# flashlight/text

Hardware: AMD Instinct MI355X
Metric: decoded frames/sec (whole node), T=1000 N=29 beam=50; hyp bit-exact vs CPU (higher is better)
Workload: dtype f64; 1 GPU; C2: LexiconFreeDecoder + ZeroLM CTC, batch=256 utterances/GPU, T=1000, N=29, beam=50, beamToken=29, beamThreshold=25, logAdd=false, `ctc` emissions; parallelism=utterance-sharded x1, no collective, threads_per_utterance=512, lds_bytes_per_workgroup=16656, engine=4, redone=0, unread_redone=0, lane_groups=1, fallback_reasons=0

## Files before the change

### text_amd/csrc/fltx_api.cpp

```cpp
#include <algorithm>
#include <cmath>
#include <cstdarg>
#include <cstdio>
#include <cstdlib>
#include <cstring>
#include <thread>
#include <limits>
#include <map>
#include <memory>
#include <mutex>
#include <string>
#include <atomic>
#include <unordered_map>
#include <unordered_set>
#include <vector>

#include "fltx.h"
#include "fltx_kernel_entry.h"
#include "fltx_engines.h"
#include "fltx_s2s.h"
#include "fltx_s2s_lex.h"
#include "fltx_ctc_rows.h"
#include "fltx_ctc_rows_lex.h"
#include "fltx_ctc_rows_stream.h"
// ... 690 lines not shown
  DBuf scored;
  HBuf hlmQCount, hlmQ, hlmBeamN, hlmBeam, hlmStage;
  DBuf hlmTabD;
  int hlmQCap = 0;
  bool hlmAnnounce = false;
  int64_t hlmAsked = 0, hlmDistinct = 0;
  bool keepScored = false;
  int64_t idCap = 0;
  DBuf tokens, words, prof, histS, bestLen, bestScores, bestTok, bestWrd;
  HBuf hTokens, hWords, hScores;
  HBuf hTok8, hWordsC, hPackMeta;
  TrBufs tr;
  HBuf hSync;
  HBuf hStat;
  DBuf dTok8, dWordsC, dPackMeta;
  std::vector<int64_t> packOff;
  bool compactFetched = false, scoresFetched = false;
  DBuf uttMap;
  int nLaunch = 0;
  std::vector<int32_t> hLen, hNHyp;
  bool hostFetched = false;
  int keepScores = 0, userKeepScores = 0;
  int profile = 0, profWave = 0;
  std::vector<int32_t> hN, hFrame, hStatus;
  bool resultsSynced = false;
  bool backtraced = false;
  int64_t statFrames = 0, statBytes = 0, statDecodeBytes = 0, statEpilogueBytes = 0, statLmBytes = 0;
  bool statsDone = false;
#ifndef FLTX_EMU
  hipEvent_t ev[3] = {nullptr, nullptr, nullptr};
  hipStream_t copyStream = nullptr;
  hipEvent_t evSlotFree[2] = {nullptr, nullptr};
  bool slotUsed[2] = {false, false};
#endif
  bool timed = false;
  struct {
    fltx_s2s_options opt{};
    int eos = 0, maxOut = 0, t = 0, cap = 0, mSel = 0, eosExtra = 0;
    bool begun = false;
    int32_t ctx0[kS2sCtx] = {0};
    DBuf beam, beamN, hist, rowsInt, done, finalStep, recTok, recAm, recN, cKey;
    DBuf scores, valid;
    DBuf recLm, lmScores;
    int lmWidth = 0, lmFinish = 0;
    DBuf rowNode, lmRowOf;
    double wordScore = 0.0;
    bool isLmToken = false;
    int maxLabels = 0, slots = 1, mSize = 0, sSize = 0, sMax = 0, maxStates = 0;
    int64_t nodes = 0, edges = 0, labels = 0, trieBytes = 0;
    DBuf trieMax, kidOff, kidTok, kidNode, labOff, lab;
    DBuf cScore, cMk, cGrp, cList, cNext, mTab, sKey, sVal, sCount, status, merges;
    int crMaxT = 0;
    int64_t crFrames = 0;
    DBuf crMeta, crEmis;
    std::vector<int64_t> crMetaHost;
    const float* crEmisDev = nullptr;
    DBuf crOutBeam;
    bool crStream = false;
    int crCap = 0, crRing = 0, crBestLb = -1;
    std::vector<int32_t> crBestLen;
    std::vector<double> crBestScores;
    DBuf crCnt, crSHist;
    DBuf crIds, crMarks;
    std::vector<int32_t> crBuf;
    bool plOn = false, plFresh = false, plSkipped = false;
    int plRowCap = 0, plMetaPar = 0, plPrevPar = 0, plCollects = 0;
    DBuf plRowOf, plFree, plMeta, plPrev, plCnt, plRank;
// ... 971 lines not shown
  d->blank = blank;
  d->unk = unk;
  d->isLmToken = isLmToken ? 1 : 0;
  if (transitions && nTrans > 0) {
    d->nTrans = nTrans;
    d->transMax = 0.0;
    for (int i = 0; i < nTrans; ++i) {
      d->transMax = std::max(d->transMax, (double)transitions[i]);
    }
    if (d->transitions.ensure(sizeof(float) * (size_t)nTrans, ctx->stream, false) ||
        devCopyH2D(d->transitions.p, transitions, sizeof(float) * (size_t)nTrans, ctx->stream) ||
        devSync(ctx->stream)) {
      delete d;
      return fail(FLTX_ERR_HIP, "transitions upload failed");
    }
  }
  *out = d;
  return FLTX_OK;
}

int fltx_decoder_destroy(fltx_decoder* d) {
  DeviceScope devScope(d ? d->ctx : nullptr);
  if (devScope.failed) {
    return fail(FLTX_ERR_HIP, "hipSetDevice failed");
  }
  if (d) {
    devSync(d->ctx->stream);
#ifndef FLTX_EMU
    for (int i = 0; i < 3; ++i) {
      if (d->ev[i]) {
        (void)hipEventDestroy(d->ev[i]);
      }
    }
    if (d->copyStream) {
      (void)hipStreamSynchronize(d->copyStream);
      (void)hipEventDestroy(d->evSlotFree[0]);
      (void)hipEventDestroy(d->evSlotFree[1]);
      (void)hipStreamDestroy(d->copyStream);
    }
#endif
  }
  delete d;
  return FLTX_OK;
}

static int settlePendingLook(fltx_decoder* d);
static int trTimedSlot(const char* key) {
  static const char* const kKeys[4] = {"transcript_count_ns", "transcript_scan_ns", "transcript_write_ns", "pack_ns"};
  for (int i = 0; i < 4; ++i) {
    if (!strcmp(key, kKeys[i])) {
      return i;
    }
  }
  return -1;
}
static int btProfileGet(fltx_decoder* d, const char* what, int64_t* value) {
  if (!d->btProfile || !d->btProf.p || !d->backtraced) {
    return fail(FLTX_ERR_STATE, "no back-trace profile: fltx_decoder_set(dec, \"bt_profile\", 1) before the batch");
  }
  DeviceScope devScope(d->ctx);
  std::vector<unsigned long long> h((size_t)kBtProfMarks * d->B);
  if (devCopyD2H(h.data(), d->btProf.p, 8 * h.size(), d->ctx->stream)) {
    return fail(FLTX_ERR_HIP, "profile copy failed");
  }
  int64_t sum[8] = {0, 0, 0, 0, 0, 0, 0, 0};
  for (int b = 0; b < d->B; ++b) {
    const unsigned long long* m = h.data() + (size_t)b * kBtProfMarks;
    if (!m[1]) {
      continue;
    }
    sum[0] += (int64_t)(m[1] - m[0]);
    unsigned long long prev = m[1];
    for (int c = 0; c < (int)m[6]; ++c) {
      sum[1] += (int64_t)(m[8 + 2 * c] - prev);
      sum[2] += (int64_t)(m[9 + 2 * c] - m[8 + 2 * c]);
      prev = m[9 + 2 * c];
    }
    sum[1] += (int64_t)(m[2] - prev);
    sum[3] += (int64_t)(m[3] - m[2]);
    if (m[5]) {
      sum[4] += (int64_t)(m[4] - m[3]);
      sum[5] += (int64_t)(m[5] - m[4]);
    }
    sum[6] += (int64_t)((m[5] ? m[5] : m[3]) - m[0]);
    sum[7] += 1;
  }
  static const char* const kNames[8] = {"copy0", "walk", "wait", "store", "fetch0", "score", "total", "utts"};
  for (int i = 0; i < 8; ++i) {
    if (!strcmp(what, kNames[i])) {
      *value = sum[i];
      return FLTX_OK;
    }
  }
  return fail(FLTX_ERR_INVALID, "fltx_decoder_get: unknown key bt_prof_%s", what);
}

int fltx_decoder_get(fltx_decoder* d, const char* key, int64_t* value) {
  if (!d || !key || !value) {
    return fail(FLTX_ERR_INVALID, "fltx_decoder_get: null argument");
  }
  if (!strcmp(key, "engine")) {
    *value = d->engineFirst;
  } else if (!strcmp(key, "xlane")) {
    *value = d->xlaneFirst;
  } else if (!strcmp(key, "ylane")) {
    *value = d->ylaneFirst;
  } else if (!strcmp(key, "yshare")) {
    *value = (d->ylane || d->xlane) ? d->yshare : 0;
  } else if (!strcmp(key, "redone")) {
    if (d->offlinePending) {
      DeviceScope devScope(d->ctx);
      int rc = settlePendingLook(d);
      if (rc) {
        return rc;
      }
    }
    *value = d->lastRedo;
  } else if (!strcmp(key, "sstream")) {
    *value = d->sstream;
  } else if (!strcmp(key, "tstream")) {
    *value = d->tstream;
// ... 1333 lines not shown
int settleStream(fltx_decoder* d);
}
static int offlineAttempts(fltx_decoder* d, const float* emissions, int32_t onDevice, int firstAttempt);
namespace {

int syncResults(fltx_decoder* d) {
  if (!d->settling && (d->chunkPending || d->pendingPrune >= 0)) {
    int rc = settleStream(d);
    if (rc) {
      return rc;
    }
  }
  if (d->offlinePending) {
    d->offlinePending = false;
    d->upSlot = d->offUpSlot;
    int rc = offlineAttempts(d, d->offEmis, 1, 1);
    if (rc) {
      return rc;
    }
  }
  if (d->resultsSynced) {
    return FLTX_OK;
  }
  Stream st = d->ctx->stream;
  const int B = d->B;
  d->hN.resize(B);
  d->hFrame.resize(B);
  d->hStatus.resize(B);
  const size_t row = d->uttRow;
  if (d->hSync.ensure(4 * (2 * row + (size_t)B))) {
    return fail(FLTX_ERR_OOM, "pinned staging allocation failed");
  }
  const int32_t* h = (const int32_t*)d->hSync.p;
  if (devCopyD2H(d->hSync.p, d->uttRes.p, 4 * (2 * row + (size_t)B), st)) {
    return fail(FLTX_ERR_HIP, "result copy failed: %s", devErr());
  }
  memcpy(d->hN.data(), h, 4 * (size_t)B);
  memcpy(d->hFrame.data(), h + row, 4 * (size_t)B);
  memcpy(d->hStatus.data(), h + 2 * row, 4 * (size_t)B);
  d->resultsSynced = true;
  return FLTX_OK;
}

int launchBacktrace(fltx_decoder* d) {
  Stream st = d->ctx->stream;
  if (d->tokens.ensure(4 * (size_t)std::max<int64_t>(d->histRecords, 1), st, false)) {
    return fail(FLTX_ERR_OOM, "token buffer allocation failed");
  }
  if (d->kind == FLTX_DECODER_LEXICON &&
      d->words.ensure(4 * (size_t)std::max<int64_t>(d->histRecords, 1), st, false)) {
    return fail(FLTX_ERR_OOM, "word buffer allocation failed");
  }
  BacktraceParams Q;
  memset(&Q, 0, sizeof(Q));
  Q.K = d->opt.beam_size;
  Q.kind = d->kind;
  Q.histPT = d->histPT.as<int2>();
  Q.histW = d->histW.as<int32_t>();
  Q.histOff = d->histOffD.as<int64_t>();
  Q.uttFrame = d->uttFrame.as<int32_t>();
  Q.uttNBeam = d->uttNBeam.as<int32_t>();
  Q.tokOff = d->histOffD.as<int64_t>();
  Q.tokens = d->tokens.as<int32_t>();
  Q.words = d->kind == FLTX_DECODER_LEXICON ? d->words.as<int32_t>() : nullptr;
  Q.nbest = 0;
#ifdef FLTX_EMU
  const int btAsked = d->btThreads ? d->btThreads : 64;
// ... 27 lines not shown
  Q.F = F;
  size_t btLds = F > 0 ? (size_t)F * perFrame + 16 : 16;
  if (d->batchPacked && F > 0) {
    Q.packed = d->packedBits;
    Q.packedTokMask = d->batchWlane ? 0x7FFFFFFF : 0xFF;
    Q.amGather = d->batchWlane ? 1 : 0;
    Q.uttStatus = d->uttStatus.as<int32_t>();
    Q.amOut = d->outScores.as<double>();
    Q.emissions = d->lastEmis;
    Q.emOff = d->emOff[d->upSlot].as<int64_t>();
    Q.N = d->N;
    Q.transitions = (d->opt.criterion == FLTX_CRITERION_ASG && d->nTrans) ? d->transitions.as<float>() : nullptr;
    Q.tokLm = d->batchTlane ? d->tokLm : nullptr;
    Q.tokLmStride = d->N + 1;
    Q.blank = d->opt.criterion == FLTX_CRITERION_CTC ? d->blank : -1;
    const size_t amLds = Q.amGather ? 4 * (size_t)Q.K * F + 16
                                    : 4 * ((size_t)F * d->N + (Q.transitions ? (size_t)d->N * d->N : 0) + (size_t)Q.K * F) + 16;
    btLds = std::max(btLds, amLds);
  }
  int narrow = 0;
  int walkWaves = 1;
  if (d->batchPacked && F > 0 && Q.K <= btThreads) {
    const bool byteRec = d->packedBits <= 8 && Q.packedTokMask == 0xFF && d->N <= 255;
    const bool wordRec = d->packedBits <= 16 && d->N <= 65535;
    const size_t rec = byteRec ? 2 : 4, tokB = rec / 2;
    size_t row = 0;
    for (int b = 0; b < d->B; ++b) {
      row = std::max<size_t>(row, (size_t)((d->histOff[b + 1] - d->histOff[b]) / Q.K));
    }
    const bool lexRec = d->kind == FLTX_DECODER_LEXICON;
    const size_t tile = ((size_t)Q.K * row * tokB + 15) & ~(size_t)15;
    const size_t room = btBudget > tile + 16 ? btBudget - tile - 16 : 0;
    const size_t perWalk = (size_t)Q.K * (2 * rec + (lexRec ? 2 * 4 + 4 : 0));
    const size_t trBytes = (Q.transitions && !Q.amGather) ? 4 * (size_t)d->N * d->N : 0;
    const size_t perEm = 2 * 4 * (size_t)d->N;
    const size_t npF = std::min<size_t>(room / perWalk, std::max<size_t>(row, 8));
    const size_t npFe = Q.amGather ? (size_t)1 << 20 : (room > trBytes ? std::min<size_t>((room - trBytes) / perEm, std::max<size_t>(row, 8)) : 0);
    const size_t nW = (size_t)btThreads / 64;
    if ((byteRec || wordRec) && Q.K <= 64 && nW >= 2 && d->btWalkAsked != 1 && row > 0 && row < (1u << 24) && npF >= 8) {
      const size_t pwChunk = (((size_t)Q.K * npF * rec + 15) & ~(size_t)15) + (lexRec ? (size_t)Q.K * npF * (4 + 4) : 0);
      const size_t exitB = (nW * Q.K + 15) & ~(size_t)15;
      const size_t ent = ((size_t)Q.K * nW * ((row + npF - 1) / npF) + 15) & ~(size_t)15;
      const size_t roomE = room > ent ? room - ent : 0;
      const size_t perEmPw = (Q.amGather ? 0 : perEm) + 2 * (size_t)Q.K * tokB;
      const size_t pwFe = roomE > trBytes ? std::min<size_t>((roomE - trBytes) / perEmPw, std::max<size_t>(row, 8)) : 0;
      if (ent + exitB + pwChunk <= room && pwFe >= 8) {
        narrow = (int)rec;
        walkWaves = (int)nW;
        Q.npRow = (int32_t)row;
        Q.npF = (int32_t)npF;
        Q.npFe = (int32_t)pwFe;
        Q.npWaves = (int32_t)nW;
        Q.npEntry = (int32_t)tile;
        Q.npScratch = (int32_t)(tile + ent);
        btLds = std::max(btLds, tile + ent + std::max(exitB + pwChunk, trBytes + pwFe * perEmPw) + 16);
      }
    }
    if (!narrow && (byteRec || wordRec) && row > 0 && row < (1u << 24) && npF >= 8 && npFe >= 8) {
      narrow = (int)rec;
      Q.npRow = (int32_t)row;
      Q.npF = (int32_t)npF;
      Q.npFe = (int32_t)npFe;
      Q.npScratch = (int32_t)tile;
      btLds = std::max(btLds, tile + std::max(npF * perWalk, Q.amGather ? (size_t)0 : trBytes + npFe * perEm) + 16);
    }
  }
  if (narrow && d->btProfile) {
    if (d->btProf.ensure(8 * (size_t)kBtProfMarks * d->B, st, true)) {
      return fail(FLTX_ERR_OOM, "back-trace profile allocation failed");
    }
    devMemset(d->btProf.p, 0, 8 * (size_t)kBtProfMarks * d->B, st);
    Q.btProf = d->btProf.as<unsigned long long>();
  }
  d->btWalkWaves = walkWaves;
  d->btNarrow = narrow;
  d->btChunk = narrow ? Q.npF : F;
  d->btStretch = narrow ? (Q.amGather ? 0 : Q.npFe) : (d->batchPacked && !Q.amGather ? F : 0);
#ifdef FLTX_EMU
  const BacktraceParams* qq = &Q;
  if (narrow == 2 && walkWaves > 1) {
    emuLaunch(d->B, btThreads, btLds, [qq](char* smem) { backtraceNarrow<uint16_t, true>(*qq, smem); });
  } else if (narrow == 4 && walkWaves > 1) {
    emuLaunch(d->B, btThreads, btLds, [qq](char* smem) { backtraceNarrow<uint32_t, true>(*qq, smem); });
  } else if (narrow == 2) {
    emuLaunch(d->B, btThreads, btLds, [qq](char* smem) { backtraceNarrow<uint16_t, false>(*qq, smem); });
  } else if (narrow == 4) {
    emuLaunch(d->B, btThreads, btLds, [qq](char* smem) { backtraceNarrow<uint32_t, false>(*qq, smem); });
  } else {
    emuLaunch(d->B, btThreads, btLds, [qq](char* smem) { backtraceUtterance(*qq, smem); });
  }
#else
  const void* btFn = narrow == 2   ? (walkWaves > 1 ? (const void*)fltx_backtrace_narrow_kernel<uint16_t, true>
                                                   : (const void*)fltx_backtrace_narrow_kernel<uint16_t, false>)
                     : narrow == 4 ? (walkWaves > 1 ? (const void*)fltx_backtrace_narrow_kernel<uint32_t, true>
                                                   : (const void*)fltx_backtrace_narrow_kernel<uint32_t, false>)
                                   : (const void*)fltx_backtrace_kernel;
  int rcLds = raiseMaxLdsOnce(d, 1, btFn, btLds);
  if (rcLds) {
    return rcLds;
  }
  void* btArgs[] = {(void*)&Q};
  HIPCHK(hipLaunchKernel(btFn, dim3(d->B), dim3(btThreads), btArgs, btLds, st));
  HIPCHK(hipGetLastError());
  if (d->ev[2]) {
    HIPCHK(hipEventRecord(d->ev[2], st));
    d->timed = true;
  }
#endif
  d->backtraced = true;
  return FLTX_OK;
// ... 445 lines not shown
    return rc;
  }
  d->lastRedo = 0;
  d->resultsSynced = false;
  if ((rc = launchBacktrace(d))) {
    return rc;
  }
  d->T.assign(T, T + B);
  d->statsDone = false;
  d->haveResults = true;
  d->ended = true;
  return FLTX_OK;
}

}

extern "C" {

int fltx_decode_batch(fltx_decoder* d, const float* emissions, int32_t onDevice, const int64_t* offsets,
                      const int32_t* T, int32_t B, int32_t N) {
  DeviceScope devScope(d ? d->ctx : nullptr);
  if (devScope.failed) {
    return fail(FLTX_ERR_HIP, "hipSetDevice failed");
  }
  if (d && stepKindCalls(d->kind)) {
    return fail(FLTX_ERR_STATE, "fltx_decode_batch: %s", stepKindCalls(d->kind));
  }
  if (!d || !T || B <= 0 || N <= 0) {
    return fail(FLTX_ERR_INVALID, "fltx_decode_batch: bad argument");
  }
  if (d->offlinePending) {
    if (d->deferCheck == 2) {
      d->offlinePending = false;
      ++d->looksDropped;
    } else {
      int rc = syncResults(d);
      if (rc) {
        return rc;
      }
      d->unreadRedone += d->lastRedo;
    }
  }
  d->streaming = false;
  d->chunkPending = false;
  d->pendingPrune = -1;
  d->haveResults = false;
  d->resultsSynced = false;
  d->backtraced = false;
  d->hostFetched = false;
  d->compactFetched = false;
  d->scoresFetched = false;
  if (d->lm->kind == 2) {
    return hostLmDecodeBatch(d, emissions, onDevice, offsets, T, B, N);
  }
  d->offT.assign(T, T + B);
  d->offOffsets.clear();
  if (offsets) {
    d->offOffsets.assign(offsets, offsets + B);
  }
  d->offN = N;
  d->offlinePending = false;
  return offlineAttempts(d, emissions, onDevice, 0);
}

}
static int settlePendingLook(fltx_decoder* d) { return syncResults(d); }
static int offlineAttempts(fltx_decoder* d, const float* emissions, int32_t onDevice, int firstAttempt) {
  const int32_t* T = d->offT.data();
  const int64_t* offsets = d->offOffsets.empty() ? nullptr : d->offOffsets.data();
  const int32_t B = (int32_t)d->offT.size(), N = d->offN;
  std::vector<int32_t> redoList;
  size_t firstRedo = 0;
  if (firstAttempt == 0) {
    d->fallbackReasons = 0;
  }
  bool recomputeRetry = false;
  bool recomputeTried = false;
  const int savedGlobalWs = d->forceGlobalWs, savedNoCut = d->noCut, savedNoLean = d->noLean, savedNoSlim = d->noSlim;
  const int savedNoSlane = d->noSlane, savedNoXlane = d->noXlane, savedNoYlane = d->noYlane, savedNoWlane = d->noWlane;
  d->offlineCall = true;
  if (firstAttempt == 0) {
    d->batchPacked = false;
    d->batchWlane = false;
    d->batchTlane = false;
  }
  d->keepScores = d->userKeepScores;
  for (int attempt = firstAttempt; attempt < 3 + firstAttempt; ++attempt) {
    const bool finalForm = attempt > firstAttempt && !recomputeRetry;
    const bool look = firstAttempt > 0 && attempt == firstAttempt;
    int rc;
    if (!look) {
      d->keepScored = attempt > 0;
      rc = prepare(d, B, N, T, finalForm);
      d->keepScored = false;
      if (rc) {
        return rc;
      }
    }
    if (!look && attempt > 0 && d->lm->kind == 1 && d->scored.p) {
// ... 95 lines not shown
        d->noCut = cut ? 1 : d->noCut;
        d->noLean = lean ? 1 : d->noLean;
        d->noSlane = slaneMiss ? 1 : d->noSlane;
        d->noWlane = wlaneMiss ? 1 : d->noWlane;
        d->noXlane = xlaneMiss ? 1 : d->noXlane;
        d->noYlane = xlaneMiss ? 1 : d->noYlane;
        d->resultsSynced = false;
        continue;
      }
    }
    break;
  }
  if (!d->offlinePending) {
    d->lastRedo = (int)firstRedo;
  }
  if (firstAttempt > 0 && firstRedo == 0) {
    return FLTX_OK;
  }
  if (firstRedo > 0 && firstRedo * 4 <= (size_t)B) {
    d->forceGlobalWs = savedGlobalWs;
    d->noCut = savedNoCut;
    d->noLean = savedNoLean;
    d->noSlim = savedNoSlim;
    d->noSlane = savedNoSlane;
    d->noWlane = savedNoWlane;
    d->noXlane = savedNoXlane;
    d->noYlane = savedNoYlane;
  }
  d->resultsSynced = false;
  int rc = launchBacktrace(d);
  if (rc) {
    return rc;
  }
  d->T.assign(T, T + B);
  d->statsDone = false;
  d->haveResults = true;
  d->ended = true;
  return FLTX_OK;
}
extern "C" {

int fltx_stream_begin(fltx_decoder* d, int32_t B, int32_t N, int32_t maxFrames) {
  DeviceScope devScope(d ? d->ctx : nullptr);
  if (devScope.failed) {
    return fail(FLTX_ERR_HIP, "hipSetDevice failed");
  }
  if (d && stepKindCalls(d->kind)) {
    return fail(FLTX_ERR_STATE, "fltx_stream_begin: %s", stepKindCalls(d->kind));
  }
  if (!d || B <= 0 || N <= 0 || maxFrames < 0) {
    return fail(FLTX_ERR_INVALID, "fltx_stream_begin: bad argument");
  }
  if (d->kind == FLTX_DECODER_LEXICON) {
    maxFrames += kLookBackLimit;
  }
  std::vector<int32_t> Tm(B, maxFrames);
  d->offlineCall = false;
  d->offlinePending = false;
  d->batchPacked = false;
  d->keepScores = 1;
  d->streamOpt = d->kind == FLTX_DECODER_LEXICON && d->userStreamOpt != 0 && !d->forceGlobalWs && d->lm->kind != 2;
  d->streamRedone = 0;
  int rc = prepare(d, B, N, Tm.data(), !d->streamOpt);
  if (rc) {
    return rc;
  }
  if (d->streamOpt && (d->lean || !(d->wsInLds || d->CAP2 > 0 || d->cutRecompute))) {
    d->streamOpt = false;
    if ((rc = prepare(d, B, N, Tm.data(), true))) {
      return rc;
    }
  }
  if (d->streamOpt &&
      d->snap.ensure((size_t)B * d->opt.beam_size * (3 * 8 + 6 * 4) + (size_t)B * 16, d->ctx->stream, false)) {
    return fail(FLTX_ERR_OOM, "stream snapshot allocation failed");
  }
  if (d->streamOpt && d->hStat.ensure(4 * (size_t)B)) {
    return fail(FLTX_ERR_OOM, "pinned status allocation failed");
  }
  latchFirst(d);
  if ((rc = bumpEpoch(d))) {
    return rc;
  }
  d->maxFrames = maxFrames;
  d->streaming = true;
  d->ended = false;
  d->haveResults = false;
  d->resultsSynced = false;
  d->backtraced = false;
  d->hostFetched = false;
  d->compactFetched = false;
// ... 1655 lines not shown
      d->histOffD.ensure(8 * ((size_t)B + 1), st, false)) {
    return fail(FLTX_ERR_OOM, "seq2seq results: device allocation failed");
  }
  if (uploadHistOff(d, st)) {
    return fail(FLTX_ERR_HIP, "seq2seq results: upload failed");
  }
  const bool lex = d->kind == FLTX_DECODER_S2S_LEXICON;
  if (lex && d->words.ensure(4 * (size_t)d->histRecords, st, false)) {
    return fail(FLTX_ERR_OOM, "seq2seq results: device allocation failed");
  }
  S2lParams Q = s2sStepParams(d);
  Q.words = lex ? d->words.as<int32_t>() : nullptr;
  S2sParams& P = Q.s;
  P.outScores = d->outScores.as<double>();
  P.tokens = d->tokens.as<int32_t>();
  P.outNHyp = d->outN.as<int32_t>();
  P.uttNBeam = d->uttNBeam.as<int32_t>();
  P.uttFrame = d->uttFrame.as<int32_t>();
  P.uttStatus = d->uttStatus.as<int32_t>();
  if (lex) {
    S2S_LAUNCH(fltx_s2s_lex_end_kernel, s2lEndUtterance, B, kS2sEndThreads, 0, st, Q);
  } else {
    S2S_LAUNCH(fltx_s2s_end_kernel, s2sEndUtterance, B, kS2sEndThreads, 0, st, P);
  }
  d->haveResults = true;
  d->ended = true;
  d->backtraced = true;
  d->streaming = false;
  d->resultsSynced = false;
  d->hostFetched = false;
  d->compactFetched = false;
  d->scoresFetched = false;
  d->offlinePending = false;
  return FLTX_OK;
}

static int crCheck(fltx_decoder* d, const char* what) {
  if (!d) {
    return fail(FLTX_ERR_INVALID, "%s: null decoder", what);
  }
  if (!isCrKind(d->kind)) {
    return fail(FLTX_ERR_STATE, "%s: not a CTC rows decoder (fltx_ctc_rows_decoder_create, "
                                "fltx_ctc_rows_lex_decoder_create)", what);
  }
  return FLTX_OK;
}

static CrParams crParams(fltx_decoder* d) {
  CrParams Q;
  memset(&Q, 0, sizeof(Q));
  S2sParams& P = Q.s;
  const int B = d->B;
  P.B = B;
  P.K = d->opt.beam_size;
  P.Kt = d->opt.beam_size_token;
  P.V = d->N;
  P.eos = -1;
  P.maxOut = std::numeric_limits<int32_t>::max();
  P.t = d->s2s.t;
  P.cap = d->s2s.cap;
  P.mSel = d->s2s.cap;
  P.beamThreshold = d->opt.beam_threshold;
  P.lmWeight = d->opt.lm_weight;
  P.beamN = d->s2s.beamN.as<int32_t>();
  P.nRowsInt = d->s2s.rowsInt.as<int32_t>();
  P.done = d->s2s.done.as<int32_t>();
// ... 582 lines not shown
                   kS2sStepThreads, sizeof(CrlStepLds), st, Z);
      } else {
        S2S_LAUNCH(fltx_ctc_rows_lex_stream_end_kernel<kCrlLmWordRows>, (crlsStepStream<kCrlLmWordRows, true>), B,
                   kS2sStepThreads, sizeof(CrlStepLds), st, Z);
      }
    } else {
      const CrStreamParams Z = {Q, crsParams(d)};
      S2S_LAUNCH(fltx_ctc_rows_stream_end_kernel, crsStepStream<true>, B, kS2sStepThreads, sizeof(S2lStepLds), st, Z);
    }
    d->s2s.crStream = false;
    d->s2s.begun = false;
    d->s2s.crBestLb = -1;
  } else if (d->kind == FLTX_DECODER_LEX_CTC_ROWS) {
    const CrlParams R = crlParams(d, Q);
    if (d->s2s.isLmToken) {
      S2S_LAUNCH(fltx_ctc_rows_lex_end_kernel<kCrlLmTokenRows>, (crlStepUtterance<kCrlLmTokenRows, true>), B,
                 kS2sStepThreads, sizeof(CrlStepLds), st, R);
    } else {
      S2S_LAUNCH(fltx_ctc_rows_lex_end_kernel<kCrlLmWordRows>, (crlStepUtterance<kCrlLmWordRows, true>), B,
                 kS2sStepThreads, sizeof(CrlStepLds), st, R);
    }
  } else {
    S2S_LAUNCH(fltx_ctc_rows_end_kernel, crStepUtterance<true>, B, kS2sStepThreads, sizeof(S2lStepLds), st, Q);
  }
  d->haveResults = true;
  d->ended = true;
  d->backtraced = true;
  d->streaming = false;
  d->resultsSynced = false;
  d->hostFetched = false;
  d->compactFetched = false;
  d->scoresFetched = false;
  d->offlinePending = false;
  return FLTX_OK;
}

static int crsCheck(fltx_decoder* d, const char* what) {
  int rc = crCheck(d, what);
  if (rc) {
    return rc;
  }
  if (!d->s2s.begun || !d->s2s.crStream) {
    return fail(FLTX_ERR_STATE, "%s: no open stream (fltx_ctc_rows_stream_begin first)", what);
  }
  return FLTX_OK;
}

static int crsReadCounts(fltx_decoder* d, std::vector<int32_t>& cnt) {
  cnt.resize(2 * (size_t)d->B);
  if (devCopyD2H(cnt.data(), d->s2s.crCnt.p, 4 * cnt.size(), d->ctx->stream) || devSync(d->ctx->stream)) {
    return fail(FLTX_ERR_HIP, "CTC rows stream: copy failed");
  }
  return FLTX_OK;
}

int fltx_ctc_rows_stream_append(fltx_decoder* d, const float* emissions, int32_t onDevice, const int64_t* offsets,
                                const int32_t* T) {
  DeviceScope devScope(d ? d->ctx : nullptr);
  if (devScope.failed) {
    return fail(FLTX_ERR_HIP, "hipSetDevice failed");
  }
  int rc = crsCheck(d, "fltx_ctc_rows_stream_append");
  if (rc) {
    return rc;
  }
  if (!T) {
// ... 620 lines not shown
```

### text_amd/csrc/fltx_kernels.h

```cpp
#pragma once
#include "fltx_rt.h"

namespace fltx {

struct TrieNodeInfo {
  float maxScore;
  int32_t labOff;
  int32_t nLabels;
  int32_t nChildren;
};

struct TrieEdge {
  int32_t child;
  float childMax;
  int32_t label0;
  uint32_t meta;
};

struct XNode {
  unsigned long long childMask;
  unsigned long long kidsMask;
  uint32_t firstChild;
  int32_t endLabel0;
  float maxScore;
// ... 3437 lines not shown
            const int tk = tT[row + j];
            if (tk >= 0) {
              if (tk != lmPrev && tk != P.blank) {
                const int2 e = P.tokLm[(size_t)lmCtx * (size_t)P.tokLmStride + (size_t)tk];
                lmAcc = lmAcc + (double)__uint_as_float((uint32_t)e.x);
                lmCtx = e.y;
              }
              lmPrev = tk;
            }
          }
        }
      }
    }
    if (tid < nh) {
      P.amOut[((size_t)b * K + tid) * 3 + 1] = am;
      if (P.tokLm) {
        lmAcc = lmAcc + (double)__uint_as_float((uint32_t)P.tokLm[(size_t)lmCtx * (size_t)P.tokLmStride + (size_t)P.N].x);
        P.amOut[((size_t)b * K + tid) * 3 + 2] = lmAcc;
      }
    }
  }
}
template <typename RT>
struct BtNarrow;
template <>
struct BtNarrow<uint16_t> {
  typedef uint8_t Tok;
};
template <>
struct BtNarrow<uint32_t> {
  typedef uint16_t Tok;
};

template <typename RT, bool PW>
FLTX_DEV void backtraceNarrow(const BacktraceParams& P, char* smem) {
  typedef typename BtNarrow<RT>::Tok TT;
  constexpr int HB = (int)sizeof(RT) * 4;
  constexpr uint32_t NONE = (1u << HB) - 1u;
  constexpr uint32_t NOROW = 0xFFu;
  const int b = (int)blockIdx.x;
  const int ff = P.uttFrame[b];
  const int len = ff + 1;
  const int L = P.npRow;
  if (!(P.uttStatus[b] & ST_PACKED) || len > L) {
    backtraceUtterance(P, smem);
    return;
  }
  const int W = (int)blockDim.x, tid = (int)threadIdx.x;
  FLTX_BT_MARK(0);
  int nh = P.uttNBeam[b];
  if (P.nbest > 0 && nh > P.nbest) {
    nh = P.nbest;
  }
  const int K = P.K;
  const bool lex = P.kind == 1;
  const int pmask = (1 << P.packed) - 1;
  const int64_t hb = P.histOff[b], ob = P.tokOff[b];
  const int F = P.npF;
  TT* tile = (TT*)smem;
  char* scr = smem + P.npScratch;
  const int nW = W >> 6, wv = tid >> 6, ln = tid & 63;
  const uint8_t* entry = (const uint8_t*)smem + P.npEntry;
  const int S = PW ? (F + nW - 1) / nW : 1;
  const float invS = 1.0f / (float)S, invF = 1.0f / (float)F;
  auto divBy = [](int d, int m, float inv) {
    int q = (int)((float)d * inv);
// ... 255 lines not shown
  if (P.btProf && tid == 0) {
    P.btProf[(size_t)b * kBtProfMarks + 6] = (unsigned long long)(c < kBtProfChunks ? c : kBtProfChunks);
  }
  for (int j0 = 0; j0 < len; j0 += 64) {
    const int j = j0 + ln;
    if (j < len) {
      const int sub = PW ? subOf(j) : 0;
      for (int k0 = wv; k0 < nh; k0 += 8 * nW) {
        uint32_t r[8];
        int t[8];
#pragma unroll
        for (int u = 0; u < 8; ++u) {
          const int k = k0 + u * nW < nh ? k0 + u * nW : k0;
          r[u] = PW ? (uint32_t)entry[(size_t)sub * K + k] : (uint32_t)k;
        }
#pragma unroll
        for (int u = 0; u < 8; ++u) {
          t[u] = tokAt(r[u], j);
        }
#pragma unroll
        for (int u = 0; u < 8; ++u) {
          const int k = k0 + u * nW;
          if (k < nh) {
            P.tokens[ob + (int64_t)k * len + j] = t[u];
          }
        }
      }
    }
  }
  FLTX_BT_MARK(3);
  if (!P.amOut) {
    return;
  }
  const int N = P.N;
  const int Fe = P.npFe;
  float* trT = (float*)scr;
  float* eT0 = trT + ((P.transitions && !P.amGather) ? (size_t)N * N : 0);
  const float* em = P.emissions + P.emOff[b];
  const float* const trG = P.amGather ? P.transitions : trT;
  const int Tb = ff - 1;
  const int aThreads = nh >= W ? W : ((nh + 63) >> 6) << 6;
  const int fThreads = W - aThreads;
  TT* hT0 = (TT*)(eT0 + (P.amGather ? 0 : (size_t)2 * Fe * N));
  auto fetch = [&](int lo, int buf, int t0, int step) {
    const int hi = lo + Fe - 1 < Tb ? lo + Fe - 1 : Tb;
    const int nEm = P.amGather ? 0 : (hi - lo + 1) * N;
    float* eT = eT0 + (size_t)buf * Fe * N;
    if (PW) {
      TT* hT = hT0 + (size_t)buf * K * Fe;
      for (int jj = t0 & 63; jj <= hi - lo; jj += 64) {
        const int sub = subOf(lo + jj);
        for (int k = t0 >> 6; k < nh; k += step >> 6) {
          const uint32_t r = entry[(size_t)sub * K + k];
          hT[k * Fe + jj] = r == NOROW ? (TT)NONE : tile[(size_t)r * L + lo + jj];
        }
      }
    }
    for (int base = t0; base < nEm; base += 8 * step) {
      float v[8];
#pragma unroll
      for (int u = 0; u < 8; ++u) {
        const int i = base + u * step;
        v[u] = i < nEm ? em[(size_t)(lo - 1) * N + i] : 0.0f;
      }
#pragma unroll
      for (int u = 0; u < 8; ++u) {
        const int i = base + u * step;
        if (i < nEm) {
          eT[i] = v[u];
        }
      }
    }
  };
  if (P.transitions && !P.amGather) {
    for (int i = tid; i < N * N; i += W) {
      trT[i] = P.transitions[i];
    }
  }
  if (Tb >= 1) {
    fetch(1, 0, tid, W);
  }
  __syncthreads();
  FLTX_BT_MARK(4);
  double am = 0.0;
  int prevTok = (tid < nh && len > 0) ? tokAt(rowOf(tid, 0), 0) : 0;
  double lmAcc = 0.0;
  int lmCtx = 0;
  int lmPrev = prevTok;
  c = 0;
  for (int lo = 1; lo <= Tb; lo += Fe, ++c) {
    const int hi = lo + Fe - 1 < Tb ? lo + Fe - 1 : Tb;
    const int nf = hi - lo + 1;
    const bool more = hi < Tb;
    const float* eT = eT0 + (size_t)(c & 1) * Fe * N;
    const TT* tokRow = PW ? hT0 + (size_t)(c & 1) * K * Fe + (size_t)tid * Fe : tile + (size_t)tid * L + lo;
    auto tokOf = [&](int jj) {
      const uint32_t t = tokRow[jj];
      return t == NONE ? -1 : (int)t;
    };
    if (tid < aThreads) {
      if (tid < nh) {
        constexpr int U = 8;
        auto walk = [&](auto withTrans) {
          constexpr bool TR = decltype(withTrans)::value;
          for (int j0 = 0; j0 < nf; j0 += U) {
            int tk[U];
            float ev[U], tr[U];
#pragma unroll
            for (int u = 0; u < U; ++u) {
              tk[u] = tokOf(j0 + u < nf ? j0 + u : nf - 1);
            }
#pragma unroll
            for (int u = 0; u < U; ++u) {
              const int jj = j0 + u < nf ? j0 + u : nf - 1;
              ev[u] = P.amGather ? em[(size_t)(lo - 1 + jj) * N + (tk[u] >= 0 ? tk[u] : 0)] : eT[jj * N + (tk[u] >= 0 ? tk[u] : 0)];
              tr[u] = 0.0f;
            }
            if (TR) {
#pragma unroll
              for (int u = 0; u < U; ++u) {
                const int pv = u == 0 ? prevTok : tk[u - 1];
                tr[u] = (tk[u] >= 0 && pv >= 0 && lo - 1 + j0 + u > 0) ? trG[(size_t)tk[u] * N + pv] : 0.0f;
              }
            }
#pragma unroll
            for (int u = 0; u < U; ++u) {
              if (j0 + u < nf && tk[u] >= 0) {
                double x = (double)ev[u];
                if (TR && lo - 1 + j0 + u > 0) {
                  x += (double)tr[u];
                }
                am += x;
                prevTok = tk[u];
              }
            }
          }
        };
        if (P.transitions) {
          walk(SlParity<1>());
        } else {
          walk(SlParity<0>());
        }
        if (P.tokLm) {
          for (int j = 0; j < nf; ++j) {
            const int tk = tokOf(j);
            if (tk >= 0) {
              if (tk != lmPrev && tk != P.blank) {
                const int2 e = P.tokLm[(size_t)lmCtx * (size_t)P.tokLmStride + (size_t)tk];
                lmAcc = lmAcc + (double)__uint_as_float((uint32_t)e.x);
                lmCtx = e.y;
              }
              lmPrev = tk;
            }
          }
        }
      }
    } else if (more) {
      fetch(hi + 1, (c + 1) & 1, tid - aThreads, fThreads);
    }
    if (more && fThreads == 0) {
      fetch(hi + 1, (c + 1) & 1, tid, W);
    }
    __syncthreads();
  }
  FLTX_BT_MARK(5);
  if (tid < nh) {
    P.amOut[((size_t)b * K + tid) * 3 + 1] = am;
    if (P.tokLm) {
      lmAcc = lmAcc + (double)__uint_as_float((uint32_t)P.tokLm[(size_t)lmCtx * (size_t)P.tokLmStride + (size_t)P.N].x);
      P.amOut[((size_t)b * K + tid) * 3 + 2] = lmAcc;
    }
  }
}

struct StreamOpParams {
  int32_t K, kind, op, lookBack;
  int2* histPT;
  int32_t* histW;
  double* histS;
  const int64_t* histOff;
  int32_t* uttFrame;
  const int32_t* uttNBeam;
  double* gScore;
  int32_t* outLen;
  double* outScores;
  int32_t* outTok;
  int32_t* outWrd;
  int32_t cap;
};

constexpr int kLookBackLimit = 100;

constexpr int kStageInts = 8192;
constexpr int kStreamOpLds = (8 + kStageInts) * 4;

FLTX_DEV void streamOpUtterance(const StreamOpParams& Q, int32_t* sh) {
  const int b = (int)blockIdx.x;
  const int tid = (int)threadIdx.x, W = (int)blockDim.x;
  const int64_t base = Q.histOff[b];
  const int ff = Q.uttFrame[b];
  const int nB = Q.uttNBeam[b];
  const int maxLookBack = Q.lookBack + kLookBackLimit;
  int32_t* stPar = sh + 8;
  int R = kStageInts / 2 / Q.K;
// ... 189 lines not shown
```

Before: 204.1 million frames/s.

## Precompute per-frame addends in LDS for backtrace scoring and queue async result copy

Reworks the narrow backtrace score pass. Stager threads now gather emission and transition values per hypothesis and frame into double-buffered LDS addend rows, where they previously staged whole emission rows. Score threads then just sum those rows with 16-byte vector loads, LM-token scoring can move to separate waves, and the next chunk is prefetched into registers. Result-summary host copies are also queued asynchronously with an event right after launch, and profiling gains add/addwait counters. The cost is more complex LDS sizing and possible summation-order changes in f64 that bit-exactness depends on.

```diff
diff --git a/text_amd/csrc/fltx_api.cpp b/text_amd/csrc/fltx_api.cpp
--- a/text_amd/csrc/fltx_api.cpp
+++ b/text_amd/csrc/fltx_api.cpp
@@ -746,7 +746,9 @@
   hipStream_t copyStream = nullptr;
   hipEvent_t evSlotFree[2] = {nullptr, nullptr};
   bool slotUsed[2] = {false, false};
+  hipEvent_t lookEv = nullptr;
 #endif
+  bool lookQueued = false;
   bool timed = false;
   struct {
     fltx_s2s_options opt{};
@@ -1784,6 +1786,9 @@
         (void)hipEventDestroy(d->ev[i]);
       }
     }
+    if (d->lookEv) {
+      (void)hipEventDestroy(d->lookEv);
+    }
     if (d->copyStream) {
       (void)hipStreamSynchronize(d->copyStream);
       (void)hipEventDestroy(d->evSlotFree[0]);
@@ -1815,7 +1820,7 @@
   if (devCopyD2H(h.data(), d->btProf.p, 8 * h.size(), d->ctx->stream)) {
     return fail(FLTX_ERR_HIP, "profile copy failed");
   }
-  int64_t sum[8] = {0, 0, 0, 0, 0, 0, 0, 0};
+  int64_t sum[10] = {0, 0, 0, 0, 0, 0, 0, 0, 0, 0};
   for (int b = 0; b < d->B; ++b) {
     const unsigned long long* m = h.data() + (size_t)b * kBtProfMarks;
     if (!m[1]) {
@@ -1833,12 +1838,14 @@
     if (m[5]) {
       sum[4] += (int64_t)(m[4] - m[3]);
       sum[5] += (int64_t)(m[5] - m[4]);
+      sum[8] += (int64_t)(m[5] - m[4]) - (int64_t)m[7];
+      sum[9] += (int64_t)m[7];
     }
     sum[6] += (int64_t)((m[5] ? m[5] : m[3]) - m[0]);
     sum[7] += 1;
   }
-  static const char* const kNames[8] = {"copy0", "walk", "wait", "store", "fetch0", "score", "total", "utts"};
-  for (int i = 0; i < 8; ++i) {
+  static const char* const kNames[10] = {"copy0", "walk", "wait", "store", "fetch0", "score", "total", "utts", "add", "addwait"};
+  for (int i = 0; i < 10; ++i) {
     if (!strcmp(what, kNames[i])) {
       *value = sum[i];
       return FLTX_OK;
@@ -3238,7 +3245,14 @@
     return fail(FLTX_ERR_OOM, "pinned staging allocation failed");
   }
   const int32_t* h = (const int32_t*)d->hSync.p;
-  if (devCopyD2H(d->hSync.p, d->uttRes.p, 4 * (2 * row + (size_t)B), st)) {
+  if (d->lookQueued) {
+    d->lookQueued = false;
+#ifndef FLTX_EMU
+    if (hipEventSynchronize(d->lookEv) != hipSuccess) {
+      return fail(FLTX_ERR_HIP, "result copy failed: %s", devErr());
+    }
+#endif
+  } else if (devCopyD2H(d->hSync.p, d->uttRes.p, 4 * (2 * row + (size_t)B), st)) {
     return fail(FLTX_ERR_HIP, "result copy failed: %s", devErr());
   }
   memcpy(d->hN.data(), h, 4 * (size_t)B);
@@ -3332,18 +3346,26 @@
     const size_t tile = ((size_t)Q.K * row * tokB + 15) & ~(size_t)15;
     const size_t room = btBudget > tile + 16 ? btBudget - tile - 16 : 0;
     const size_t perWalk = (size_t)Q.K * (2 * rec + (lexRec ? 2 * 4 + 4 : 0));
-    const size_t trBytes = (Q.transitions && !Q.amGather) ? 4 * (size_t)d->N * d->N : 0;
-    const size_t perEm = 2 * 4 * (size_t)d->N;
+    const size_t trBytes = (Q.transitions && !Q.amGather) ? btTransBytes(d->N) : 0;
     const size_t npF = std::min<size_t>(room / perWalk, std::max<size_t>(row, 8));
-    const size_t npFe = Q.amGather ? (size_t)1 << 20 : (room > trBytes ? std::min<size_t>((room - trBytes) / perEm, std::max<size_t>(row, 8)) : 0);
+    const bool withTrans = Q.transitions != nullptr;
+    auto stretchFor = [&](size_t avail, bool tokRows) {
+      const size_t perFe = (size_t)2 * Q.K * (withTrans ? 8 : 4) + (tokRows ? (size_t)2 * Q.K * tokB : 0);
+      size_t fe = std::min<size_t>(avail / perFe, std::max<size_t>(row, 8));
+      while (fe > 0 && btScoreBytes(Q.K, (int)fe, withTrans, tokRows, (int)tokB) > avail) {
+        --fe;
+      }
+      return fe;
+    };
+    const size_t npFe = room > trBytes ? stretchFor(room - trBytes, false) : 0;
     const size_t nW = (size_t)btThreads / 64;
     if ((byteRec || wordRec) && Q.K <= 64 && nW >= 2 && d->btWalkAsked != 1 && row > 0 && row < (1u << 24) && npF >= 8) {
       const size_t pwChunk = (((size_t)Q.K * npF * rec + 15) & ~(size_t)15) + (lexRec ? (size_t)Q.K * npF * (4 + 4) : 0);
       const size_t exitB = (nW * Q.K + 15) & ~(size_t)15;
       const size_t ent = ((size_t)Q.K * nW * ((row + npF - 1) / npF) + 15) & ~(size_t)15;
       const size_t roomE = room > ent ? room - ent : 0;
-      const size_t perEmPw = (Q.amGather ? 0 : perEm) + 2 * (size_t)Q.K * tokB;
-      const size_t pwFe = roomE > trBytes ? std::min<size_t>((roomE - trBytes) / perEmPw, std::max<size_t>(row, 8)) : 0;
+      const bool tokRows = Q.tokLm != nullptr;
+      const size_t pwFe = roomE > trBytes ? stretchFor(roomE - trBytes, tokRows) : 0;
       if (ent + exitB + pwChunk <= room && pwFe >= 8) {
         narrow = (int)rec;
         walkWaves = (int)nW;
@@ -3353,7 +3375,7 @@
         Q.npWaves = (int32_t)nW;
         Q.npEntry = (int32_t)tile;
         Q.npScratch = (int32_t)(tile + ent);
-        btLds = std::max(btLds, tile + ent + std::max(exitB + pwChunk, trBytes + pwFe * perEmPw) + 16);
+        btLds = std::max(btLds, tile + ent + std::max(exitB + pwChunk, trBytes + btScoreBytes(Q.K, (int)pwFe, withTrans, tokRows, (int)tokB)) + 16);
       }
     }
     if (!narrow && (byteRec || wordRec) && row > 0 && row < (1u << 24) && npF >= 8 && npFe >= 8) {
@@ -3362,7 +3384,7 @@
       Q.npF = (int32_t)npF;
       Q.npFe = (int32_t)npFe;
       Q.npScratch = (int32_t)tile;
-      btLds = std::max(btLds, tile + std::max(npF * perWalk, Q.amGather ? (size_t)0 : trBytes + npFe * perEm) + 16);
+      btLds = std::max(btLds, tile + std::max(npF * perWalk, trBytes + btScoreBytes(Q.K, (int)npFe, withTrans, false, (int)tokB)) + 16);
     }
   }
   if (narrow && d->btProfile) {
@@ -3375,7 +3397,7 @@
   d->btWalkWaves = walkWaves;
   d->btNarrow = narrow;
   d->btChunk = narrow ? Q.npF : F;
-  d->btStretch = narrow ? (Q.amGather ? 0 : Q.npFe) : (d->batchPacked && !Q.amGather ? F : 0);
+  d->btStretch = narrow ? Q.npFe : (d->batchPacked && !Q.amGather ? F : 0);
 #ifdef FLTX_EMU
   const BacktraceParams* qq = &Q;
   if (narrow == 2 && walkWaves > 1) {
@@ -3887,6 +3909,7 @@
   if (d->offlinePending) {
     if (d->deferCheck == 2) {
       d->offlinePending = false;
+      d->lookQueued = false;
       ++d->looksDropped;
     } else {
       int rc = syncResults(d);
@@ -3920,6 +3943,23 @@
 
 }
 static int settlePendingLook(fltx_decoder* d) { return syncResults(d); }
+static int queueLook(fltx_decoder* d) {
+#ifndef FLTX_EMU
+  const size_t bytes = 4 * (2 * d->uttRow + (size_t)d->B);
+  if (d->hSync.ensure(bytes)) {
+    return fail(FLTX_ERR_OOM, "pinned staging allocation failed");
+  }
+  if (!d->lookEv) {
+    HIPCHK(hipEventCreateWithFlags(&d->lookEv, hipEventDisableTiming));
+  }
+  HIPCHK(hipMemcpyAsync(d->hSync.p, d->uttRes.p, bytes, hipMemcpyDeviceToHost, d->ctx->stream));
+  HIPCHK(hipEventRecord(d->lookEv, d->ctx->stream));
+  d->lookQueued = true;
+#else
+  (void)d;
+#endif
+  return FLTX_OK;
+}
 static int offlineAttempts(fltx_decoder* d, const float* emissions, int32_t onDevice, int firstAttempt) {
   const int32_t* T = d->offT.data();
   const int64_t* offsets = d->offOffsets.empty() ? nullptr : d->offOffsets.data();
@@ -4081,6 +4121,10 @@
   if (rc) {
     return rc;
   }
+  d->lookQueued = false;
+  if (d->offlinePending && (rc = queueLook(d))) {
+    return rc;
+  }
   d->T.assign(T, T + B);
   d->statsDone = false;
   d->haveResults = true;
@@ -4106,6 +4150,7 @@
   std::vector<int32_t> Tm(B, maxFrames);
   d->offlineCall = false;
   d->offlinePending = false;
+  d->lookQueued = false;
   d->batchPacked = false;
   d->keepScores = 1;
   d->streamOpt = d->kind == FLTX_DECODER_LEXICON && d->userStreamOpt != 0 && !d->forceGlobalWs && d->lm->kind != 2;
@@ -5827,6 +5872,7 @@
   d->compactFetched = false;
   d->scoresFetched = false;
   d->offlinePending = false;
+  d->lookQueued = false;
   return FLTX_OK;
 }
 
@@ -6475,6 +6521,7 @@
   d->compactFetched = false;
   d->scoresFetched = false;
   d->offlinePending = false;
+  d->lookQueued = false;
   return FLTX_OK;
 }
 
diff --git a/text_amd/csrc/fltx_kernels.h b/text_amd/csrc/fltx_kernels.h
--- a/text_amd/csrc/fltx_kernels.h
+++ b/text_amd/csrc/fltx_kernels.h
@@ -3493,6 +3493,30 @@
   typedef uint16_t Tok;
 };
 
+template <bool TR>
+struct BtAddend;
+template <>
+struct BtAddend<false> {
+  typedef float T;
+  struct alignas(16) Quad {
+    float v[4];
+  };
+};
+template <>
+struct BtAddend<true> {
+  typedef double T;
+  struct alignas(16) Quad {
+    double v[2];
+  };
+};
+constexpr int btAddStride(int Fe, int per) {
+  return ((((Fe + per - 1) / per) & 1) ? (Fe + per - 1) / per : (Fe + per - 1) / per + 1) * per;
+}
+constexpr size_t btTransBytes(int N) { return ((size_t)4 * N * N + 15) & ~(size_t)15; }
+constexpr size_t btScoreBytes(int K, int Fe, bool withTrans, bool tokRows, int tokBytes) {
+  return (size_t)2 * K * btAddStride(Fe, withTrans ? 2 : 4) * (withTrans ? 8 : 4) + (tokRows ? (size_t)2 * K * Fe * tokBytes : 0);
+}
+
 template <typename RT, bool PW>
 FLTX_DEV void backtraceNarrow(const BacktraceParams& P, char* smem) {
   typedef typename BtNarrow<RT>::Tok TT;
@@ -3814,144 +3838,261 @@
   if (!P.amOut) {
     return;
   }
+  if (nh <= 0) {
+    return;
+  }
   const int N = P.N;
   const int Fe = P.npFe;
+  const float* em = P.emissions + P.emOff[b];
+  const int Tb = ff - 1;
+  const bool trLds = P.transitions && !P.amGather;
   float* trT = (float*)scr;
-  float* eT0 = trT + ((P.transitions && !P.amGather) ? (size_t)N * N : 0);
-  const float* em = P.emissions + P.emOff[b];
+  char* addB = scr + (trLds ? btTransBytes(N) : 0);
   const float* const trG = P.amGather ? P.transitions : trT;
-  const int Tb = ff - 1;
-  const int aThreads = nh >= W ? W : ((nh + 63) >> 6) << 6;
-  const int fThreads = W - aThreads;
-  TT* hT0 = (TT*)(eT0 + (P.amGather ? 0 : (size_t)2 * Fe * N));
-  auto fetch = [&](int lo, int buf, int t0, int step) {
-    const int hi = lo + Fe - 1 < Tb ? lo + Fe - 1 : Tb;
-    const int nEm = P.amGather ? 0 : (hi - lo + 1) * N;
-    float* eT = eT0 + (size_t)buf * Fe * N;
-    if (PW) {
-      TT* hT = hT0 + (size_t)buf * K * Fe;
-      for (int jj = t0 & 63; jj <= hi - lo; jj += 64) {
-        const int sub = subOf(lo + jj);
-        for (int k = t0 >> 6; k < nh; k += step >> 6) {
-          const uint32_t r = entry[(size_t)sub * K + k];
-          hT[k * Fe + jj] = r == NOROW ? (TT)NONE : tile[(size_t)r * L + lo + jj];
-        }
-      }
-    }
-    for (int base = t0; base < nEm; base += 8 * step) {
-      float v[8];
-#pragma unroll
-      for (int u = 0; u < 8; ++u) {
-        const int i = base + u * step;
-        v[u] = i < nEm ? em[(size_t)(lo - 1) * N + i] : 0.0f;
-      }
-#pragma unroll
-      for (int u = 0; u < 8; ++u) {
-        const int i = base + u * step;
-        if (i < nEm) {
-          eT[i] = v[u];
-        }
-      }
-    }
-  };
-  if (P.transitions && !P.amGather) {
+  if (trLds) {
     for (int i = tid; i < N * N; i += W) {
       trT[i] = P.transitions[i];
     }
-  }
-  if (Tb >= 1) {
-    fetch(1, 0, tid, W);
-  }
-  __syncthreads();
-  FLTX_BT_MARK(4);
+    __syncthreads();
+  }
+  const int aThreads = nh >= W ? W : ((nh + 63) >> 6) << 6;
+  const bool lmWaves = P.tokLm && W - aThreads >= 2 * aThreads;
+  const int sBase = aThreads + (lmWaves ? aThreads : 0);
+  const int fThreads = W - sBase;
+  const int kL = lmWaves ? tid - aThreads : tid;
+  const bool lmMine = P.tokLm && kL >= 0 && kL < nh;
+  auto tokKJ = [&](int k, int j) { return tokAt(rowOf(k, j), j); };
   double am = 0.0;
-  int prevTok = (tid < nh && len > 0) ? tokAt(rowOf(tid, 0), 0) : 0;
   double lmAcc = 0.0;
   int lmCtx = 0;
-  int lmPrev = prevTok;
-  c = 0;
-  for (int lo = 1; lo <= Tb; lo += Fe, ++c) {
-    const int hi = lo + Fe - 1 < Tb ? lo + Fe - 1 : Tb;
-    const int nf = hi - lo + 1;
-    const bool more = hi < Tb;
-    const float* eT = eT0 + (size_t)(c & 1) * Fe * N;
-    const TT* tokRow = PW ? hT0 + (size_t)(c & 1) * K * Fe + (size_t)tid * Fe : tile + (size_t)tid * L + lo;
-    auto tokOf = [&](int jj) {
-      const uint32_t t = tokRow[jj];
-      return t == NONE ? -1 : (int)t;
+  int lmPrev = (lmMine && len > 0) ? tokKJ(kL, 0) : 0;
+  unsigned long long waitAcc = 0;
+  auto scorePass = [&](auto withTrans) {
+    constexpr bool TR = decltype(withTrans)::value;
+    typedef typename BtAddend<TR>::T AT;
+    typedef typename BtAddend<TR>::Quad Quad;
+    constexpr int PER = 16 / (int)sizeof(AT);
+    constexpr int PF = 3;
+    const int stride = btAddStride(Fe, PER);
+    AT* add0 = (AT*)addB;
+    TT* hT0 = (TT*)(addB + (size_t)2 * K * stride * sizeof(AT));
+    const bool stager = fThreads > 0 && tid >= sBase;
+    struct Lay {
+      int cols, G, jj, kq;
     };
-    if (tid < aThreads) {
-      if (tid < nh) {
-        constexpr int U = 8;
-        auto walk = [&](auto withTrans) {
-          constexpr bool TR = decltype(withTrans)::value;
-          for (int j0 = 0; j0 < nf; j0 += U) {
-            int tk[U];
-            float ev[U], tr[U];
-#pragma unroll
-            for (int u = 0; u < U; ++u) {
-              tk[u] = tokOf(j0 + u < nf ? j0 + u : nf - 1);
+    auto layFor = [&](int t, int nT) {
+      Lay y;
+      y.cols = stride < nT ? stride : nT;
+      y.G = nT / y.cols;
+      y.jj = t % y.cols;
+      y.kq = t / y.cols < y.G ? t / y.cols : (1 << 24);
+      return y;
+    };
+    const Lay layAll = layFor(tid, W);
+    const Lay laySt = stager ? layFor(tid - sBase, fThreads) : layAll;
+    const bool ahead = stager && stride <= fThreads;
+    auto tokVia = [&](const uint8_t* entRow, int k, int j) {
+      const uint32_t row = PW ? (uint32_t)entRow[k] : (uint32_t)k;
+      const bool none = PW && row == NOROW;
+      const uint32_t t = tile[(size_t)(none ? 0u : row) * L + j];
+      return (none || t == NONE) ? -1 : (int)t;
+    };
+    auto gather = [&](const uint8_t* e0, const uint8_t* e1, int k, int j, int jj, float& ev, float& tr) -> bool {
+      const int tk = tokVia(e0, k, j);
+      ev = em[(size_t)(j - 1) * N + (tk >= 0 ? tk : 0)];
+      tr = 0.0f;
+      if (TR) {
+        int pv = tokVia(e1, k, j - 1);
+        if (jj == 0) {
+          for (int p = j - 2; pv < 0 && p >= 0; --p) {
+            pv = tokKJ(k, p);
+          }
+        }
+        const float t = trG[(size_t)(tk >= 0 ? tk : 0) * N + (pv >= 0 ? pv : 0)];
+        tr = (tk >= 0 && pv >= 0) ? t : 0.0f;
+      }
+      return tk >= 0;
+    };
+    auto addend = [&](bool on, float ev, float tr, int j) -> AT {
+      if constexpr (TR) {
+        double x = (double)ev;
+        if (j > 1) {
+          x += (double)tr;
+        }
+        return on ? x : -0.0;
+      } else {
+        return on ? ev : -0.0f;
+      }
+    };
+    auto direct = [&](int lo, int buf, const Lay& y, int skip) {
+      const int hi = lo + Fe - 1 < Tb ? lo + Fe - 1 : Tb;
+      const int nf = hi - lo + 1;
+      AT* A = add0 + (size_t)buf * K * stride;
+      if (y.kq + skip * y.G >= nh) {
+        return;
+      }
+      for (int jj = y.jj; jj < ((nf + PER - 1) & ~(PER - 1)); jj += y.cols) {
+        const bool inF = jj < nf;
+        const int j = lo + (inF ? jj : 0);
+        const uint8_t* e0 = entry + (PW ? (size_t)subOf(j) * K : 0);
+        const uint8_t* e1 = entry + ((PW && TR) ? (size_t)subOf(j - 1) * K : 0);
+        for (int k0 = y.kq + skip * y.G; k0 < nh; k0 += PF * y.G) {
+          float ev[PF], tr[PF];
+          bool on[PF];
+#pragma unroll
+          for (int u = 0; u < PF; ++u) {
+            const int k = k0 + u * y.G;
+            on[u] = gather(e0, e1, k < nh ? k : 0, j, jj, ev[u], tr[u]) && inF;
+          }
+#pragma unroll
+          for (int u = 0; u < PF; ++u) {
+            const int k = k0 + u * y.G;
+            if (k < nh) {
+              A[k * stride + jj] = addend(on[u], ev[u], tr[u], j);
             }
-#pragma unroll
-            for (int u = 0; u < U; ++u) {
-              const int jj = j0 + u < nf ? j0 + u : nf - 1;
-              ev[u] = P.amGather ? em[(size_t)(lo - 1 + jj) * N + (tk[u] >= 0 ? tk[u] : 0)] : eT[jj * N + (tk[u] >= 0 ? tk[u] : 0)];
-              tr[u] = 0.0f;
+          }
+        }
+      }
+    };
+    struct Held {
+      float ev[PF], tr[PF];
+      uint32_t on;
+    };
+    Held hA = {{0.0f, 0.0f, 0.0f}, {0.0f, 0.0f, 0.0f}, 0u}, hB = hA;
+    auto issue = [&](int lo, const Lay& y, Held& h) {
+      const int hi = lo + Fe - 1 < Tb ? lo + Fe - 1 : Tb;
+      const int nf = hi - lo + 1;
+      h.on = 0;
+      const bool inF = y.jj < nf;
+      const int j = lo + (inF ? y.jj : 0);
+      const uint8_t* e0 = entry + (PW ? (size_t)subOf(j) * K : 0);
+      const uint8_t* e1 = entry + ((PW && TR) ? (size_t)subOf(j - 1) * K : 0);
+#pragma unroll
+      for (int u = 0; u < PF; ++u) {
+        const int k = y.kq + u * y.G;
+        h.on |= ((gather(e0, e1, k < nh ? k : 0, j, inF ? y.jj : 1, h.ev[u], h.tr[u]) && inF) ? 1u : 0u) << u;
+      }
+    };
+    auto put = [&](int lo, int buf, const Lay& y, const Held& h) {
+      const int hi = lo + Fe - 1 < Tb ? lo + Fe - 1 : Tb;
+      const int nf = hi - lo + 1;
+      AT* A = add0 + (size_t)buf * K * stride;
+      if (y.jj < ((nf + PER - 1) & ~(PER - 1))) {
+#pragma unroll
+        for (int u = 0; u < PF; ++u) {
+          const int k = y.kq + u * y.G;
+          if (k < nh) {
+            A[k * stride + y.jj] = addend((h.on >> u) & 1u, h.ev[u], h.tr[u], lo + y.jj);
+          }
+        }
+      }
+    };
+    auto stageTok = [&](int lo, int buf, int t0, int step) {
+      if (PW && P.tokLm) {
+        const int hi = lo + Fe - 1 < Tb ? lo + Fe - 1 : Tb;
+        TT* hT = hT0 + (size_t)buf * K * Fe;
+        for (int jj = t0 & 63; jj <= hi - lo; jj += 64) {
+          const int sub = subOf(lo + jj);
+          for (int k = t0 >> 6; k < nh; k += step >> 6) {
+            const uint32_t r = entry[(size_t)sub * K + k];
+            hT[k * Fe + jj] = r == NOROW ? (TT)NONE : tile[(size_t)r * L + lo + jj];
+          }
+        }
+      }
+    };
+    if (Tb >= 1) {
+      direct(1, 0, layAll, 0);
+      stageTok(1, 0, tid, W);
+      if (ahead) {
+        issue(1 + Fe <= Tb ? 1 + Fe : 1, laySt, hA);
+      }
+    }
+    __syncthreads();
+    FLTX_BT_MARK(4);
+    auto round = [&](int lo, int c, Held& cur, Held& nxt) {
+      const int hi = lo + Fe - 1 < Tb ? lo + Fe - 1 : Tb;
+      const int nf = hi - lo + 1;
+      const bool more = hi < Tb;
+      if (tid < aThreads && tid < nh) {
+        const Quad* R = (const Quad*)(add0 + (size_t)(c & 1) * K * stride + (size_t)tid * stride);
+        const int nq = (nf + PER - 1) / PER;
+        Quad q0 = R[0], q1 = R[nq > 1 ? 1 : 0];
+        for (int q = 0; q < nq; q += 2) {
+          const Quad n0 = R[q + 2 < nq ? q + 2 : nq - 1], n1 = R[q + 3 < nq ? q + 3 : nq - 1];
+#pragma unroll
+          for (int u = 0; u < PER; ++u) {
+            am += (double)q0.v[u];
+          }
+          if (q + 1 < nq) {
+#pragma unroll
+            for (int u = 0; u < PER; ++u) {
+              am += (double)q1.v[u];
             }
-            if (TR) {
-#pragma unroll
-              for (int u = 0; u < U; ++u) {
-                const int pv = u == 0 ? prevTok : tk[u - 1];
-                tr[u] = (tk[u] >= 0 && pv >= 0 && lo - 1 + j0 + u > 0) ? trG[(size_t)tk[u] * N + pv] : 0.0f;
-              }
+          }
+          q0 = n0;
+          q1 = n1;
+        }
+      }
+      if (lmMine && (tid < aThreads || lmWaves)) {
+        const TT* tokRow = PW ? hT0 + (size_t)(c & 1) * K * Fe + (size_t)kL * Fe : tile + (size_t)kL * L + lo;
+        for (int j = 0; j < nf; ++j) {
+          const uint32_t t = tokRow[j];
+          if (t != NONE) {
+            const int tk = (int)t;
+            if (tk != lmPrev && tk != P.blank) {
+              const int2 e = P.tokLm[(size_t)lmCtx * (size_t)P.tokLmStride + (size_t)tk];
+              lmAcc = lmAcc + (double)__uint_as_float((uint32_t)e.x);
+              lmCtx = e.y;
             }
-#pragma unroll
-            for (int u = 0; u < U; ++u) {
-              if (j0 + u < nf && tk[u] >= 0) {
-                double x = (double)ev[u];
-                if (TR && lo - 1 + j0 + u > 0) {
-                  x += (double)tr[u];
-                }
-                am += x;
-                prevTok = tk[u];
-              }
-            }
-          }
-        };
-        if (P.transitions) {
-          walk(SlParity<1>());
-        } else {
-          walk(SlParity<0>());
-        }
-        if (P.tokLm) {
-          for (int j = 0; j < nf; ++j) {
-            const int tk = tokOf(j);
-            if (tk >= 0) {
-              if (tk != lmPrev && tk != P.blank) {
-                const int2 e = P.tokLm[(size_t)lmCtx * (size_t)P.tokLmStride + (size_t)tk];
-                lmAcc = lmAcc + (double)__uint_as_float((uint32_t)e.x);
-                lmCtx = e.y;
-              }
-              lmPrev = tk;
-            }
-          }
-        }
-      }
-    } else if (more) {
-      fetch(hi + 1, (c + 1) & 1, tid - aThreads, fThreads);
-    }
-    if (more && fThreads == 0) {
-      fetch(hi + 1, (c + 1) & 1, tid, W);
-    }
-    __syncthreads();
+            lmPrev = tk;
+          }
+        }
+      }
+      if (more) {
+        const int nb = (c + 1) & 1;
+        if (stager) {
+          direct(hi + 1, nb, laySt, ahead ? PF : 0);
+          stageTok(hi + 1, nb, tid - sBase, fThreads);
+          if (ahead) {
+            issue(hi + 1 + Fe <= Tb ? hi + 1 + Fe : hi + 1, laySt, nxt);
+            put(hi + 1, nb, laySt, cur);
+          }
+        } else if (fThreads == 0) {
+          direct(hi + 1, nb, layAll, 0);
+          stageTok(hi + 1, nb, tid, W);
+        }
+      }
+      unsigned long long tw = 0;
+      if (P.btProf && tid == 0) {
+        tw = devClock();
+      }
+      ldsBarrier();
+      if (P.btProf && tid == 0) {
+        waitAcc += devClock() - tw;
+      }
+    };
+    for (int lo = 1, c = 0; lo <= Tb; lo += 2 * Fe, c += 2) {
+      round(lo, c, hA, hB);
+      if (lo + Fe <= Tb) {
+        round(lo + Fe, c + 1, hB, hA);
+      }
+    }
+  };
+  if (P.transitions) {
+    scorePass(SlParity<1>());
+  } else {
+    scorePass(SlParity<0>());
   }
   FLTX_BT_MARK(5);
+  if (P.btProf && tid == 0) {
+    P.btProf[(size_t)b * kBtProfMarks + 7] = waitAcc;
+  }
   if (tid < nh) {
     P.amOut[((size_t)b * K + tid) * 3 + 1] = am;
-    if (P.tokLm) {
-      lmAcc = lmAcc + (double)__uint_as_float((uint32_t)P.tokLm[(size_t)lmCtx * (size_t)P.tokLmStride + (size_t)P.N].x);
-      P.amOut[((size_t)b * K + tid) * 3 + 2] = lmAcc;
-    }
+  }
+  if (lmMine && (tid < aThreads || lmWaves)) {
+    lmAcc = lmAcc + (double)__uint_as_float((uint32_t)P.tokLm[(size_t)lmCtx * (size_t)P.tokLmStride + (size_t)P.N].x);
+    P.amOut[((size_t)b * K + kL) * 3 + 2] = lmAcc;
   }
 }
 
```

Result: faster. 214.8 million frames/s (median of 6 runs) (+5.2%).
